# astooke/accel_rl

Measured on AMD Instinct MI355X. Metric: env-steps/sec (whole node), 256-env PPO Atari, higher is better.
Workload: dtype f32; 1 GPU; PPO breakout, 256 envs/GPU, horizon 5, spec-1 CNN (fp32), minibatch 512/GPU x 4 epochs, adam; synthetic fixed-frame emulator; hipGraph rollout; total_envs=256, global_minibatch=512, parallelism=single

## Files before the change

### accel_rl_amd/_lib.py

```python
import ctypes as C
import os

import torch

_PKG = os.path.dirname(os.path.abspath(__file__))
LIB_PATH = os.path.join(_PKG, "libaccel_rl_hip.so")

ARL_ABI_VERSION = 4
PROMO_NEP50, PROMO_LEGACY, PROMO_ASSOC = 0, 1, 2
PPO_TIE_THEANO, PPO_TIE_MATH, PPO_TIE_BOTH = 0, 1, 2
OPT_ADAM, OPT_RMSPROP = 0, 1
MAX_ACTIONS = 18
REPLAY_MAX_HORIZON = 16
RAW_H, RAW_W, OBS_H, OBS_W = 210, 160, 104, 80
OPT_PARTIALS = 1024

_vp, _i32, _i64, _f32, _f64 = C.c_void_p, C.c_int32, C.c_int64, C.c_float, C.c_double


class ArlGame(C.Structure):
    _fields_ = [("bank", _vp), ("n_frames", _i32), ("n_actions", _i32),
                ("action_set", _i32 * MAX_ACTIONS), ("start_lives", _i32),
                ("life_period", _i32), ("frame_skip", _i32), ("n_stack", _i32),
                ("clip_reward", _i32), ("episodic_lives", _i32), ("resample_mode", _i32)]
# ... 37 lines not shown
    _fields_ = [("part", _vp), ("out", _vp), ("total", _i64), ("splits", _i32), ("valid", _i32)]


FOLD_MAX_ITEMS = 24


class ArlLogitSrc(C.Structure):
    _fields_ = [("part", _vp), ("bias_or_null", _vp), ("split_stride", _i64), ("splits", _i32), ("reserved", _i32)]


class ArlDgradWt(C.Structure):
    _fields_ = [("w", _vp), ("wt", _vp), ("geom", C.POINTER(ArlConvGeom))]


DGRAD_WT_MAX = 4


class ArlServeHead(C.Structure):
    _fields_ = [("hidden", ArlFoldItem), ("hidden_bias", _vp), ("hidden_relu", _i32), ("hid", _i32),
                ("w_head", _vp), ("b_head", _vp)]


class ArlServeConv1(C.Structure):
    _fields_ = [("geom", C.POINTER(ArlConvGeom)), ("w", _vp), ("bias", _vp), ("y", _vp), ("scale", _f32),
                ("relu", _i32)]


class ArlNoisyLayer(C.Structure):
    _fields_ = [("fein", _vp), ("feout", _vp), ("x", _vp), ("xs", _vp), ("fan_in", _i32), ("units", _i32),
                ("out_stride", _i32), ("layer", _i32)]
# ... 38 lines not shown
    "arl_sample_categorical": (_i32, [_vp, _vp, _i64, _i32, _vp, _vp]),
    "arl_env_act_step": (_i32, [C.POINTER(ArlGame), C.POINTER(ArlEnvState), C.POINTER(ArlRollout),
                                _vp, _vp, _vp, _vp, _i32, _i32, _f64, _f64, _vp]),
    "arl_env_frame_step": (_i32, [C.POINTER(ArlGame), C.POINTER(ArlEnvState), C.POINTER(ArlRollout),
                                  _i32, _i32, _vp]),
    "arl_env_step": (_i32, [C.POINTER(ArlGame), C.POINTER(ArlEnvState), C.POINTER(ArlRollout),
                            _vp, _vp, _vp, _vp, _i32, _i32, _f64, _f64, _i32, _i32, _vp]),
    "arl_rollout_begin": (_i32, [C.POINTER(ArlGame), C.POINTER(ArlEnvState), C.POINTER(ArlRollout), _vp]),
    "arl_env_reset": (_i32, [C.POINTER(ArlGame), C.POINTER(ArlEnvState), C.POINTER(ArlRollout),
                             _vp, _i32, _vp]),
    "arl_preprocess_frames": (_i32, [_vp, _vp, _i64, _i32, _vp, _vp]),
    "arl_copy_bytes": (_i32, [_vp, _vp, _i64, _vp]),
    "arl_ring_append": (_i32, [_vp, _i32, _vp, _i32, _vp, _vp]),
    "arl_gather_scale_obs": (_i32, [_vp, _vp, _i64, _i64, _f32, _vp, _vp]),
    "arl_gather_scale_obs_nhwc": (_i32, [_vp, _vp, _i64, _i32, _i32, _f32, _vp, _vp]),
    "arl_traj_minibatch": (_i32, [_vp, _i32, _i32, _i64, C.POINTER(_vp), _i32, _i32, _vp, _vp, C.POINTER(_vp), _vp, _vp]),
    "arl_bias_relu": (_i32, [_vp, _vp, _i64, _i32, _vp]),
    "arl_relu_bwd_workspace_bytes": (_i64, []),
    "arl_relu_bwd_bias_grad": (_i32, [_vp, _vp, _i64, _i32, _vp, _vp, _vp]),
    "arl_pg_head_workspace_bytes": (_i64, []),
    "arl_pg_head_infer": (_i32, [_vp, _vp, _vp, _i64, _i32, _i32, _vp, _vp, _vp]),
    "arl_pg_head_loss": (_i32, [_vp] * 11 + [_i64, _i32, _i32, _i32, _i32, _f32, _f32, _f32, _i32] + [_vp] * 7),
    "arl_pg_head_loss_parts": (_i32, [_vp] * 11 + [_i64, _i32, _i32, _i32, _i32, _f32, _f32, _f32, _i32] + [_vp] * 7 +
                               [_vp, _i32, _vp]),
    "arl_conv_workspace_bytes": (_i64, []),
    "arl_conv2d_fwd": (_i32, [_vp, _vp, _vp, _vp, C.POINTER(ArlConvGeom), _i32, _vp, _vp]),
    "arl_conv2d_bwd_data": (_i32, [_vp, _vp, _vp, _vp, _vp, C.POINTER(ArlConvGeom), C.POINTER(ArlCorunJob), C.POINTER(_i32), _vp]),
    "arl_conv2d_dgrad_weights": (_i32, [C.POINTER(ArlDgradWt), _i32, _vp]),
    "arl_conv2d_bwd_weight": (_i32, [_vp, _vp, _vp, C.POINTER(ArlConvGeom), _vp, _vp]),
    "arl_conv2d_bwd_weight_parts": (_i32, [_vp, _vp, _vp, C.POINTER(ArlConvGeom), _vp, _i64, C.POINTER(ArlFoldItem),
# ... 349 lines not shown


def gather_scale_obs_nhwc(obs, idx, out, scale, stream=None):
    _want(obs, torch.uint8, "obs")
    _want(out, torch.float32, "out")
    if idx is not None:
        _want(idx, torch.int32, "idx")
    batch = out.shape[0]
    channels, plane = obs.shape[1], obs.shape[2] * obs.shape[3]
    assert out.numel() == batch * channels * plane
    _check(load().arl_gather_scale_obs_nhwc(ptr(obs), ptr(idx), batch, channels, plane, float(scale),
                                            out.data_ptr(), stream_ptr(stream)),
           "arl_gather_scale_obs_nhwc")


def traj_minibatch(seg, horizon, state_in, valids, idx, state_out, inv_count=None, stream=None):
    _want(seg, torch.int32, "seg")
    _want(idx, torch.int32, "idx")
    n_seg, n_state = seg.numel(), len(state_in)
    if len(state_out) != n_state:
        raise ValueError("traj_minibatch: %d states in, %d out" % (n_state, len(state_out)))
    if idx.numel() != n_seg * horizon:
        raise ValueError("traj_minibatch: idx holds %d rows, not %d segments x %d" % (idx.numel(), n_seg, horizon))
    hidden, total = 0, None
    for a, b in zip(state_in, state_out):
        _want(a, torch.float32, "state_in")
        _want(b, torch.float32, "state_out")
        hidden = a.shape[-1]
        if b.numel() != n_seg * hidden or a.numel() % (hidden * horizon) or total not in (None, a.numel() // hidden):
            raise ValueError("traj_minibatch: state shapes %s -> %s" % (tuple(a.shape), tuple(b.shape)))
# ... 649 lines not shown
```

### accel_rl_amd/algos/pg/aac_base.py

```python
import torch

from accel_rl_amd import _lib
from accel_rl_amd.algos.base import RLAlgorithm
from accel_rl_amd.buffers import buffer_with_segs_view
from accel_rl_amd.util import logger
from accel_rl_amd.util.misc import graph_capture_mode
from accel_rl_amd.util.quick_args import save_args
import numpy as np

LR_SCHEDULES = ["linear"]


def valids_mean(expression, valids=None):
    if valids is None:
        return expression.mean()
    v = valids.to(expression.dtype)
    return torch.sum(v * expression) * (1. / torch.sum(v))


class AdvActorCriticBase(RLAlgorithm):

    def __init__(self, discount, gae_lambda, v_loss_coeff=1, ent_loss_coeff=0.01,
                 standardize_adv=False, lr_schedule=None, promo="nep50", use_graph=True, bptt_resets=False):
        if lr_schedule is not None and lr_schedule not in LR_SCHEDULES:
# ... 41 lines not shown
            raise TypeError("the policy must provide loss_and_grads (HIP forward / backward into its flat "
                            "gradient bucket); got {}".format(type(policy).__name__))
        extra = dict(horizon=horizon, data_length=sample_size) if traj_opt else dict()
        self.optimizer.initialize(inputs=input_names, losses=self._losses, constraints=None, target=policy,
                                  lr_mult=self._lr_mult, **extra)
        self._opt_buf = buffer_with_segs_view(opt_examples, sample_size, horizon, dev)
        self._batch_size = sample_size
        self._mid_batch_reset = mid_batch_reset
        self._horizon = horizon
        self._n_env = sample_size // horizon
        self._std_ws = _lib.standardize_workspace(dev)
        self._lr_mult_host = torch.ones(1, dtype=torch.float32).pin_memory()
        self._graph = None
        self._graph_out = None
        self._graph_samples = None
        self._warm_calls = 0
        self._done_event = None
        self._info_ring = None
        self._info_replays = 0

    def set_n_itr(self, n_itr):
        self.n_itr = n_itr

    def optimize_policy(self, itr, samples_data):
        if self._done_event is not None:
            self._done_event.synchronize()
        if self.lr_schedule == "linear":
            self._lr_mult_host.fill_(max((self.n_itr - itr) / self.n_itr, 0.))
        if hasattr(self.optimizer, "prepare_host"):
            self.optimizer.prepare_host(self._batch_size)
# ... 5 lines not shown

    def _enqueue_optimize(self, itr, samples_data):
        tag = self.optimizer.parallelism_tag
        sync = tag == "synchronous" and getattr(self.optimizer, "graph_ready", lambda: False)()
        graphable = self.use_graph and hasattr(self.optimizer, "device_updates") and (tag == "single" or sync)
        if not graphable:
            return self._device_optimize(itr, samples_data)
        if self._graph is None:
            self._warm_calls += 1
            if self._warm_calls <= 2:
                out = self._device_optimize(itr, samples_data)
                self._ensure_info_ring(out[1])
                return out
            torch.cuda.synchronize(self.policy.device)
            graph, failure = torch.cuda.CUDAGraph(), None
            opt_host = {k: getattr(self.optimizer, k) for k in
                        ("_n_updates", "_hole", "_call_hole", "_hole_count", "_pending_avg") if hasattr(self.optimizer, k)}
            try:
                with torch.cuda.graph(graph, capture_error_mode=graph_capture_mode()):
                    self._graph_out = self._device_optimize(itr, samples_data)
                    self._append_infos(self._graph_out[1])
            except Exception as e:
                if not sync:
                    raise
                failure = e
            if sync and not self.optimizer.ranks_agree(failure is None):
                logger.log("WARNING: hipGraph capture of the synchronous learner failed on a rank (%r): eager "
                           "minibatches from here on" % (failure,))
                self.optimizer.graph_collectives = False
                for k, v in opt_host.items():
                    setattr(self.optimizer, k, v)
                torch.cuda.synchronize(self.policy.device)
                return self._device_optimize(itr, samples_data)
            self._graph, self._graph_samples = graph, samples_data
        assert samples_data is self._graph_samples, "the sampler must hand over the same buffer"
        self._graph.replay()
        opt_data, infos = self._graph_out
        slot = self._info_replays % next(iter(self._info_ring.values())).shape[0]
        self._info_replays += 1
        return opt_data, {k: self._info_ring[k][slot] for k in infos}

    INFO_RING = 4096
    _log_interval_itrs = 0

    def set_log_interval_itrs(self, n):
        self._log_interval_itrs = int(n)
        ring = getattr(self, "_info_ring", None)
        if ring is not None and self._ring_slots() > next(iter(ring.values())).shape[0]:
            raise RuntimeError("set_log_interval_itrs(%d) after the diagnostics ring was sized" % n)

    def _ring_slots(self):
        return max(self.INFO_RING, self._log_interval_itrs + 2)

    def _ensure_info_ring(self, infos):
        if self._info_ring is None:
# ... 77 lines not shown
```

### accel_rl_amd/csrc/batch_ops.hip

```cpp

#include <stdarg.h>
#include <string.h>

#include "arl_common.h"

namespace arl {
static thread_local char g_err[512] = "";
void set_error(const char* fmt, ...) {
    va_list ap;
    va_start(ap, fmt);
    vsnprintf(g_err, sizeof(g_err), fmt, ap);
    va_end(ap);
}
}

extern "C" int arl_abi_version(void) { return ARL_ABI_VERSION; }
extern "C" const char* arl_last_error(void) { return arl::g_err; }

namespace {

constexpr int STD_BLOCKS = 512;

__device__ __forceinline__ double wave_sum(double x) {
#pragma unroll
// ... 76 lines not shown
    const int64_t stride = (int64_t)gridDim.x * blockDim.x;
    for (int64_t i = (int64_t)blockIdx.x * blockDim.x + threadIdx.x; i < total; i += stride) {
        const int64_t b = i / row_vec, q = i - b * row_vec;
        const int64_t src_row = idx ? (int64_t)idx[b] : b;
        const uint4 w = reinterpret_cast<const uint4*>(obs)[src_row * row_vec + q];
        const uint32_t ws[4] = {w.x, w.y, w.z, w.w};
        float4* o = reinterpret_cast<float4*>(out) + i * 4;
#pragma unroll
        for (int k = 0; k < 4; ++k) {
            o[k] = make_float4((float)(ws[k] & 255u) * scale, (float)((ws[k] >> 8) & 255u) * scale,
                               (float)((ws[k] >> 16) & 255u) * scale, (float)(ws[k] >> 24) * scale);
        }
    }
}

}

extern "C" int64_t arl_standardize_workspace_bytes(void) { return (int64_t)STD_BLOCKS * 3 * sizeof(double); }

extern "C" int arl_standardize(float* advantages, const int8_t* valids_or_null, int64_t n,
                               double eps, void* workspace, void* stream) {
    ARL_REQUIRE(advantages && workspace, ARL_E_ARG, "null pointer");
    ARL_REQUIRE(n >= 0, ARL_E_ARG, "negative n");
    if (n == 0) return 0;
    hipStream_t s = (hipStream_t)stream;
    int64_t nb = (n + 255) / 256;
    if (nb > STD_BLOCKS) nb = STD_BLOCKS;
    hipLaunchKernelGGL(moments_kernel, dim3((unsigned)nb), dim3(256), 0, s, advantages,
                       valids_or_null, n, (double*)workspace);
    int rc = arl::check_launch("moments_kernel");
// ... 64 lines not shown
    return arl::check_launch("copy_kernel");
}

extern "C" int arl_gather_scale_obs(const uint8_t* obs, const int32_t* idx_or_null, int64_t batch,
                                    int64_t row_bytes, float scale, float* out, void* stream) {
    ARL_REQUIRE(obs && out, ARL_E_ARG, "null pointer");
    ARL_REQUIRE(batch >= 0 && row_bytes > 0, ARL_E_ARG, "bad batch/row_bytes");
    ARL_REQUIRE((row_bytes & 15) == 0, ARL_E_RANGE, "row_bytes must be a multiple of 16");
    ARL_REQUIRE(arl::aligned16(obs) && arl::aligned16(out), ARL_E_ALIGN, "obs/out must be 16-byte aligned");
    if (batch == 0) return 0;
    const int64_t row_vec = row_bytes >> 4;
    hipLaunchKernelGGL(gather_scale_kernel, dim3(arl::stream_grid(batch * row_vec, 256)), dim3(256),
                       0, (hipStream_t)stream, obs, idx_or_null, batch, row_vec, scale, out);
    return arl::check_launch("gather_scale_kernel");
}
```

### accel_rl_amd/optimizers/base.py

```python
import numpy as np
import torch

from accel_rl_amd import _lib

NORM_LOG_LEN = 64


def iterate_mb_idxs(batch_size, data_length, shuffle=False):
    if shuffle:
        order = np.arange(data_length)
        np.random.shuffle(order)
    for lo in range(0, data_length - batch_size + 1, batch_size):
        yield order[lo:lo + batch_size] if shuffle else np.arange(lo, lo + batch_size)


def iterate_traj_idxs(batch_size, data_length, horizon=1, shuffle=False):
    if data_length % horizon or batch_size % horizon or data_length % batch_size:
        raise AssertionError("batch_size and data_length must be multiples of horizon, data_length of batch_size")
    rows = np.arange(data_length).reshape(-1, horizon)
    order = np.arange(data_length // horizon)
    per = batch_size // horizon
    if shuffle:
        np.random.shuffle(order)
    for lo in range(0, len(order), per):
# ... 34 lines not shown
        st = _lib.ArlOptState()
        st.n_params = n
        st.params, st.grads = target.flat_params.data_ptr(), target.flat_grads.data_ptr()
        st.slot0 = self._slot0.data_ptr()
        st.slot1 = self._slot1.data_ptr() if self._slot1 is not None else None
        st.step_count, st.lr_mult = self._step_count.data_ptr(), self._lr_mult.data_ptr()
        st.partials, st.grad_norm_log = self._partials.data_ptr(), self._norm_log.data_ptr()
        st.norm_log_len = NORM_LOG_LEN
        self._opt_state = st
        a = self._update_args
        if self._update_method.name == "adam":
            self._kernel_args = (a["beta1"], a["beta2"], a["epsilon"])
        else:
            self._kernel_args = (a["rho"], 0.0, a["epsilon"])

    def _backward(self, losses, minibatch):
        return losses(minibatch)[3]

    def _apply_update(self, avg_factor=1.0):
        b1, b2, eps = self._kernel_args
        if self._grad_norm_clip is None:
            self._noclip_state()
            k = self._n_updates % self._opt_state.norm_log_len
            hole, self._hole = self._hole, None
            if k == 0:
                self._call_hole = hole
                self._hole_count = hole[1] if hole else 0
            elif self._hole_count and hole is None:
                hole = self._call_hole
                _lib.corun_job_run(_lib.corun_job(self._opt_state, self._update_method.kernel_id, self._learning_rate,
                                                  avg_factor, b1, b2, eps, k, self._step_pp, self._norm_parts,
                                                  hole[0], hole[1]))
            if self._hole_count:
                hole = self._call_hole
                _lib.opt_step_noclip_split(self._opt_state, self._update_method.kernel_id, self._learning_rate,
                                           avg_factor, b1, b2, eps, k, self._step_pp, self._norm_parts, hole[0],
                                           hole[1], 0)
            else:
                _lib.opt_step_noclip(self._opt_state, self._update_method.kernel_id, self._learning_rate, avg_factor,
                                     b1, b2, eps, k, self._step_pp, self._norm_parts)
            self._pending_avg = avg_factor
        else:
            _lib.opt_step(self._opt_state, self._update_method.kernel_id, self._learning_rate,
                          avg_factor, self._grad_norm_clip, b1, b2, eps)
        self._n_updates += 1

    corun_update = True

    def _noclip_state(self):
        if self._step_pp is None:
            dev = self._target.device
            self._step_pp = self._step_count.repeat(2).contiguous()
            self._norm_parts = torch.zeros(_lib.OPT_NORM_SLOTS * _lib.OPT_NORM_BLOCKS, dtype=torch.float64, device=dev)
        elif self._n_updates % self._opt_state.norm_log_len == 0 and not self._hole:
            self._step_pp.copy_(self._step_count.expand(2))

    def _corun_hook(self, avg_factor=1.0):
        if self._grad_norm_clip is not None or not self.corun_update:
            return None
        b1, b2, eps = self._kernel_args
# ... 28 lines not shown
```

### accel_rl_amd/optimizers/single.py

```python
import numpy as np
import torch

from accel_rl_amd import _lib

from accel_rl_amd.optimizers.base import BaseOptimizer, iterate_mb_idxs, iterate_traj_idxs


class A2cOptimizer(BaseOptimizer):

    def __init__(self, learning_rate, update_method, update_method_args=None, grad_norm_clip=None):
        self._learning_rate = learning_rate
        self._update_method = update_method
        self._update_args = update_method.resolve(**(update_method_args or dict()))
        self._grad_norm_clip = grad_norm_clip

    def initialize(self, inputs, losses, constraints, target, givens=None, lr_mult=1):
        self._input_names = list(inputs)
        self._losses = losses
        self._setup_bucket(target, lr_mult, givens)

    def optimize(self, inputs):
        self.prepare_host(len(inputs[0]))
        return self.device_updates(inputs)

    def prepare_host(self, data_length):
        self._set_updates_per_call(1)

    def device_updates(self, inputs):
        minibatch = dict(zip(self._input_names, inputs))
        minibatch["idx"] = None
        loss = self._backward(self._losses, minibatch)
        self._share_grad()
        self._apply_update(self._avg_factor())
        return loss, self._recent_grad_norms(1)

    def _share_grad(self):
        pass

    def _avg_factor(self):
        return 1.0

    @property
    def parallelism_tag(self):
        return "single"

# ... 33 lines not shown
        if flat:
            self._idx_host.copy_(torch.from_numpy(np.stack(flat).astype(np.int32)))

    def device_updates(self, inputs):
        data = dict(zip(self._input_names, inputs))
        if not self._n_minibatches:
            return [], []
        _lib.copy_bytes(self._idx_dev, self._idx_host)
        if self._overlap_allreduce:
            return self._overlapped_minibatches(data)
        losses = []
        corun = self._corun_hook() if self.parallelism_tag == "single" else None
        try:
            for k in range(self._n_minibatches):
                mb = self._minibatch(data, self._idx_dev[k])
                if corun is not None:
                    mb["dense_w_hook"] = corun
                losses.append(self._backward(self._losses, mb))
                self._share_grad()
                self._apply_update(self._avg_factor())
        finally:
            self._hole = None
        return losses, self._recent_grad_norms(self._n_minibatches)

    def _minibatch(self, data, idx):
        return dict(data, idx=idx)

    _overlap_allreduce = False

    def _overlapped_minibatches(self, data):
# ... 80 lines not shown
```

### accel_rl_amd/policies/atari_cnn_policy.py

```python
import ctypes as C
import os

import numpy as np
import torch

from accel_rl_amd import _lib
from accel_rl_amd.distributions import Categorical
from accel_rl_amd.spaces import Discrete
from accel_rl_amd.util.seed import layer_rng

KIND_A2C, KIND_PPO = 0, 1


def _glorot_uniform(shape):
    receptive = int(np.prod(shape[2:]))
    fan_in, fan_out = shape[1] * receptive, shape[0] * receptive
    a = np.sqrt(6. / (fan_in + fan_out))
    return layer_rng().uniform(low=-a, high=a, size=shape).astype(np.float32)


def _norm_c(shape, std):
    out = np.random.randn(*shape).astype(np.float32)
    out *= std / np.sqrt(np.square(out).sum(axis=0, keepdims=True))
    return out


class ObsRows(object):
    __slots__ = ("obs", "idx", "shape")

    def __init__(self, obs, idx):
        self.obs, self.idx = obs.contiguous(), idx
        self.shape = (obs.shape[0] if idx is None else idx.shape[0],) + tuple(obs.shape[1:])


class AtariCnnPolicy(object):

    _u8_conv1 = True
    serves_rows = True

    def __init__(self, conv_filters, conv_filter_sizes, conv_strides, conv_pads,
                 hidden_sizes=(), pixel_scale=255., initial_param_values=None):
        self.conv_filters, self.conv_filter_sizes = list(conv_filters), list(conv_filter_sizes)
        self.conv_strides, self.conv_pads = list(conv_strides), list(conv_pads)
        self.hidden_sizes = list(hidden_sizes)
        if not self.hidden_sizes:
            raise NotImplementedError("at least one hidden dense layer is required")
        self.pixel_scale = pixel_scale
# ... 61 lines not shown
        def views(flat):
            out = []
            for k, (o, n, s) in enumerate(zip(self._offsets, sizes, shapes)):
                v = flat[o:o + n].view(s)
                out.append(v.permute(0, 3, 1, 2) if (len(s) == 4 and not (k == 0 and self._u8)) else v)
            return out
        self.params = [torch.nn.Parameter(v) for v in views(self.flat_params)]
        self.grads = views(self.flat_grads)
        self._w = [self.flat_params[o:o + n] for o, n in zip(self._offsets, sizes)]
        self._g = [self.flat_grads[o:o + n] for o, n in zip(self._offsets, sizes)]
        self._conv_ws = _lib.conv_workspace(self.device)
        self._wt = {i: torch.empty_like(self._w[2 * i]) for i, (nf, ci, sz, st, pad, ho, wo) in enumerate(self._conv_geom)
                    if i > 0 and 16 < ci <= 64 and st <= 2 and sz % st == 0 and
                    os.environ.get("ARL_DGRAD_WT", "1") != "0"}
        self._geoms = dict()
        for p, g in zip(self.params, self.grads):
            p.grad = g
        self._n_conv, self._n_hid = len(self._conv_geom), len(self._hid_geom)
        self._dist = Categorical(n_act)
        self._scale = float(np.float32(1. / self.pixel_scale))
        self._relu_ws = _lib.relu_bwd_workspace(self.device)
        self._folds, self._fold_workspaces = _lib.FoldList(), {}
        self._loss_ws = _lib.pg_head_workspace(self.device)
        self._set_from_reference_arrays(ref)
        if self.initial_param_values is not None:
            self.set_param_values(self.initial_param_values)

    def _hidden_reference_init(self, fan):
        ref, names, self._hid_geom = [], [], []
        for i, hs in enumerate(self.hidden_sizes):
# ... 127 lines not shown

    def prob_value(self, observations, rows=None):
        with torch.no_grad():
            x = self._scaled(observations, rows)
            b = x.shape[0]
            _, hids = self._trunk(x)
            prob = torch.empty((b, self.n_act), dtype=torch.float32, device=self.device)
            value = torch.empty(b, dtype=torch.float32, device=self.device)
            _lib.pg_head_infer(hids[-1], self.params[-2], self.params[-1], prob, value)
            return prob, value

    def serve_supported(self):
        return (type(self).prob_value is AtariCnnPolicy.prob_value and self._n_hid >= 1 and
                self._hid_geom[-1][0] <= 1024 and self.n_act <= _lib.MAX_ACTIONS)

    def serve_conv1(self, game, b):
        conv_g, _ = self._layer_geoms(b)
        if not (self._u8 and _lib.serve_conv1_supported(game, conv_g[0])):
            return None, None
        nf, ci, sz, st, pad, ho, wo = self._conv_geom[0]
        y1 = self._buffer(("act", 0, b), (b, ho, wo, nf))
        conv1 = _lib.ArlServeConv1()
        conv1.geom = C.pointer(conv_g[0])
        conv1.w, conv1.bias, conv1.y = self._w[0].data_ptr(), self._w[1].data_ptr(), y1.data_ptr()
        conv1.scale, conv1.relu = self._scale, 1
        return conv1, y1

    def serve_forward(self, game, observations, rows, y1=None, want_next=True):
        with torch.no_grad():
            b = rows.shape[0]
            conv_g, dense_g = self._layer_geoms(b)
            w = self._w
            nf, ci, sz, st, pad, ho, wo = self._conv_geom[0]
            if y1 is None:
                x = self._scaled(observations, rows)
                y1 = self._buffer(("act", 0, b), (b, ho, wo, nf))
                if isinstance(x, ObsRows):
                    _lib.conv2d_u8_fwd(x.obs, x.idx, self._scale, w[0], w[1], y1, conv_g[0], True)
                else:
                    _lib.conv2d_fwd(x, w[0], w[1], y1, conv_g[0], True, self._conv_ws)
            a = y1
            for i in range(1, self._n_conv):
                nf_i, _, _, _, _, ho_i, wo_i = self._conv_geom[i]
                z = self._buffer(("act", i, b), (b, ho_i, wo_i, nf_i))
                _lib.conv2d_fwd(a, w[2 * i], w[2 * i + 1], z, conv_g[i], True, self._conv_ws)
                a = z
            k = 2 * self._n_conv
            for j, (hs, fan_in) in enumerate(self._hid_geom):
                hcur = self._buffer(("hid", j, b), (b, hs))
                if j + 1 < self._n_hid:
                    _lib.conv2d_fwd(a, w[k], w[k + 1], hcur, dense_g[j], True, self._conv_ws)
                else:
                    item = _lib.conv2d_fwd_parts(a, w[k], w[k + 1], hcur, dense_g[j], True, self._conv_ws)
                a = hcur
                k += 2
            head = _lib.ArlServeHead()
            head.hidden = item
            head.hidden_bias, head.hidden_relu, head.hid = w[k - 1].data_ptr(), 1, self._hid_geom[-1][0]
            head.w_head, head.b_head = w[self._k_head].data_ptr(), w[self._k_head + 1].data_ptr()
            conv1 = None
            if want_next and self._u8 and _lib.serve_conv1_supported(game, conv_g[0]):
                conv1 = _lib.ArlServeConv1()
                conv1.geom = C.pointer(conv_g[0])
                conv1.w, conv1.bias, conv1.y = w[0].data_ptr(), w[1].data_ptr(), y1.data_ptr()
                conv1.scale, conv1.relu = self._scale, 1
            return head, conv1, (y1 if conv1 is not None else None)

    def loss_and_grads(self, mb, kind, clip_param, v_loss_coeff, ent_loss_coeff, lr_mult,
                       inv_count=None, tie_rule=_lib.PPO_TIE_THEANO):
        with torch.no_grad():
            idx = mb.get("idx")
            rows = mb["observations"].shape[0] if idx is None else idx.shape[0]
            limit = self.rows_per_pass()
            if limit and rows >= 3 * limit:
                return self._loss_and_grads_in_passes(mb, rows, limit, kind, clip_param, v_loss_coeff, ent_loss_coeff,
                                                      lr_mult, inv_count, tie_rule)
            x = self._scaled(mb["observations"], idx)
            b = x.shape[0]
            acts, hids = self._trunk(x)
            g, k_head = self.grads, self._k_head
            hid = self._hid_geom[-1][0]
            dout = self._buffer(("dout", b), (b, self.n_act + 1))
            dh = self._buffer(("dh", b), (b, hid))
            loss4 = self._buffer(("loss", b), (4,))
            wts = self._dgrad_weight_items(b) if os.environ.get("ARL_WT_IN_HEAD", "1") != "0" else []
            self._folds.pg_head_loss(hids[-1], self.params[k_head], self.params[k_head + 1], mb["actions"],
                              mb["advantages"], mb["returns"], mb.get("old_prob"), mb.get("valids"),
                              idx, lr_mult, inv_count, self.n_act, kind, clip_param, v_loss_coeff,
                              ent_loss_coeff, dout, dh, g[k_head], g[k_head + 1], loss4, self._loss_ws,
                              relu_mask_dh=True, tie_rule=tie_rule, dgrad_weights=wts)
            self._wt_fresh = bool(wts)
            try:
                self._backward_trunk(x, acts, hids, dh, masked=True, split_hook=mb.get("split_hook"),
                                     dense_w_hook=mb.get("dense_w_hook"))
# ... 178 lines not shown
        for i in range(self._n_conv):
            w = ref[k][:, :, ::-1, ::-1]
            if not (i == 0 and self._u8):
                w = w.transpose(0, 2, 3, 1)
            if i == 0 and not self._u8 and self._c_pad != self._c_in:
                w = np.concatenate([w, np.zeros(w.shape[:3] + (self._c_pad - self._c_in,), np.float32)], axis=3)
            internal += [w, ref[k + 1]]
            k += 2
        tail = self._tail_from_flat(list(ref[k:]))
        internal += self._hidden_to_internal(tail[:self._n_hidden_tensors])
        internal += self._head_to_internal(tail[self._n_hidden_tensors:])
        for o, s, a in zip(self._offsets, self._shapes, internal):
            assert tuple(a.shape) == tuple(s), (a.shape, s)
            host[o:o + a.size] = np.ascontiguousarray(a).reshape(-1)
        self.flat_params.copy_(torch.from_numpy(host))

    def set_param_values(self, flat, trainable=True):
        flat = np.asarray(flat, np.float32)
        assert flat.size == self.n_params
        ref, pos = [], 0
        for s in self._ref_shapes:
            n = int(np.prod(s))
            ref.append(flat[pos:pos + n].reshape(s))
            pos += n
        self._set_from_reference_arrays(ref)
```

### accel_rl_amd/runners/sync.py

```python
import os
import time

import torch
import torch.distributed as dist

from accel_rl_amd.runners.accel_rl import AccelRL
from accel_rl_amd.util import logger


class AccelRLSync(AccelRL):

    def __init__(self, affinities=None, seed=None, backend=None, **kwargs):
        self._backend = backend
        self._worker_affinities = None
        self._worker_procs = []
        as_list = list(affinities) if isinstance(affinities, (list, tuple)) else None
        if "WORLD_SIZE" in os.environ:
            self.rank = int(os.environ.get("RANK", 0))
            self.n_runners = int(os.environ["WORLD_SIZE"])
            if as_list is not None:
                if len(as_list) != self.n_runners:
                    raise ValueError("AccelRLSync got %d affinities but WORLD_SIZE=%d: one entry per launched rank "
                                     "(multigpu_rl_base.py:21)" % (len(as_list), self.n_runners))
                affinities = as_list[self.rank]
# ... 134 lines not shown
        n_itr = super().startup(master=True)
        self.init_comm()
        self._start_time = self._last_time = time.time()
        return n_itr

    def init_comm(self):
        if self.n_runners > 1:
            n = torch.tensor([self.policy.flat_params.numel()], dtype=torch.int64, device=self.policy.flat_params.device)
            lo, hi = n.clone(), n.clone()
            dist.all_reduce(lo, op=dist.ReduceOp.MIN)
            dist.all_reduce(hi, op=dist.ReduceOp.MAX)
            if int(lo) != int(hi):
                raise ValueError("AccelRLSync: the runners' policies differ in size (%d ... %d parameters, %d here): a "
                                 "synchronous clique all-reduces ONE flat bucket" % (int(lo), int(hi), int(n)))
            dist.broadcast(self.policy.flat_params, src=0)
            self._initial_param_vector = self.policy.flat_params.clone()
        self.algo.optimizer.init_comm(None, self.rank, self.n_runners)
        if self.n_runners > 1:
            dist.barrier()

    def get_n_itr(self, sample_size):
        n_itr = super().get_n_itr(sample_size * self.n_runners)
        return n_itr

    def store_diagnostics(self, itr, samples_data, opt_data, traj_infos, opt_infos):
        if self.n_runners > 1 and (itr + 1) % self._log_interval_itrs == 0:
            pending = getattr(self, "_pending_traj", []) + list(traj_infos)
            gathered = [None] * self.n_runners
            dist.all_gather_object(gathered, [dict(t) for t in pending])
            self._pending_traj = []
# ... 16 lines not shown
```

### accel_rl_amd/sampler/gpu_sampler.py

```python
import ctypes
import os

import numpy as np
import torch

from accel_rl_amd import _lib
from accel_rl_amd.buffers import (buffer_with_segs_view, batch_buffer, combine_distinct_buffers,
                                  buffer_length, count_buffer_size)
from accel_rl_amd.envs import synthetic_atari as synth
from accel_rl_amd.sampler.base import BaseMbSampler
from accel_rl_amd.sampler.util import TrajInfo
from accel_rl_amd.util import logger
from accel_rl_amd.util.misc import graph_capture_mode, nbytes_unit, struct

NOOP_RING = 4096


def _packed_block(spec, device, pinned=False):
    offsets, total = [], 0
    for _, shape, dtype in spec:
        total = (total + 127) // 128 * 128
        offsets.append(total)
        total += int(np.prod(shape)) * torch.empty((), dtype=dtype).element_size()
    block = torch.zeros(total, dtype=torch.uint8, device=device)
# ... 41 lines not shown
    def __eq__(self, other):
        self.resolve()
        return super().__eq__(other)

    def __repr__(self):
        self.resolve()
        return super().__repr__()


class GpuVecSampler(BaseMbSampler):

    _alias_extra_obs = True
    _serve_in_step = os.environ.get("ARL_SERVE_IN_STEP", "1") != "0"
    _serve_in_step_max_envs = (512, 1024)
    _two_host_sets = os.environ.get("ARL_TWO_HOST_SETS", "1") != "0"

    def __init__(self, n_parallel=1, envs_per=1, device=None, use_graph=True, **kwargs):
        super().__init__(n_parallel=n_parallel, envs_per=envs_per, **kwargs)
        self._total_n_envs = 2 * n_parallel * envs_per
        self.device = device
        self.use_graph = use_graph
        self._sets, self._batch_no = [], 0

    @property
    def _graph(self):
        return self._sets[0].graph if self._sets else None

    @_graph.setter
    def _graph(self, value):
        for h in self._sets:
# ... 133 lines not shown
                agent_infos[key] = np.zeros(state.shape[1], np.float32)
            self._prev_frozen = torch.zeros(n, dtype=torch.uint8, device=dev)
        examples = dict(actions=np.zeros((), self.env_spec.action_space.dtype), agent_infos=agent_infos)
        policy_buf = buffer_with_segs_view(examples, n * t, t, dev)
        self.samples_buf = combine_distinct_buffers(self.envs_buf, policy_buf)
        assert buffer_length(self.samples_buf) == self.sample_size
        policy.reset(n_batch=n if self._recurrent else self.n_parallel * self.envs_per)
        self._rollout = self._make_rollout(self.samples_buf)
        self._single_write = bool(self.mid_batch_reset and not self._recurrent and
                                  getattr(policy, "serves_rows", False) and self._kernel_max_path_length() >= 1)
        self._serve_fused = bool(self._single_write and type(self)._serve_in_step and self._game.n_stack <= 4 and
                                 hasattr(policy, "serve_forward") and policy.serve_supported())
        if self._serve_fused:
            with_conv1 = policy.serve_conv1(self._game, n)[0] is not None
            self._serve_fused = n <= type(self)._serve_in_step_max_envs[int(with_conv1)]
        self._extra_is_step_obs = bool(self.need_extra_obs and self.mid_batch_reset and type(self)._alias_extra_obs)
        if self._extra_is_step_obs:
            self.samples_buf.extra_observations = self.envs_buf.extra_observations = self.step_obs
        self._step_rows = (torch.arange(n, dtype=torch.int32, device=dev)[None, :] * t +
                           torch.arange(t, dtype=torch.int32, device=dev)[:, None]).contiguous()
        self._uniforms = torch.empty((t, n), dtype=torch.float64, device=dev)
        self._sets, self._batch_no, self._last_pending = [], 0, None
        overlap = (self.use_graph and type(self)._two_host_sets and not hasattr(policy, "host_draws") and not self._recurrent)
        for _ in range(2 if overlap else 1):
            block, views = _packed_block(self._results_spec, "cpu", pinned=True)
            self._sets.append(struct(uniforms_host=torch.empty(t * n, dtype=torch.float64).pin_memory(), host_block=block,
                                     host=struct(**views), event=torch.cuda.Event(), pending=None, graph=None))
        logger.log("GpuVecSampler -- total_n_envs: {}".format(self.total_n_envs))
        logger.log("GpuVecSampler -- batch buffer size: {:,.1f} {}".format(
            *nbytes_unit(count_buffer_size(self.samples_buf))))
# ... 2 lines not shown
        n, t = self._total_n_envs, self.horizon
        cur = self._sets[self._batch_no % len(self._sets)]
        self._batch_no += 1
        if cur.pending is not None:
            cur.pending.resolve()
        draws = self.policy.host_draws(t, n) if hasattr(self.policy, "host_draws") else np.random.rand(t * n)
        cur.uniforms_host.copy_(torch.from_numpy(draws))
        with torch.cuda.device(self.device):
            if self.use_graph:
                if cur.graph is None:
                    self._capture(cur)
                cur.graph.replay()
            else:
                self._enqueue_batch(cur)
            cur.event.record()
        older = self._last_pending if (self._last_pending is not None and self._last_pending._sampler is not None) else None
        cur.pending = self._last_pending = _LazyTrajInfos(self, cur, older)
        return self.samples_buf, cur.pending

    def shutdown(self):
        for h in self._sets:
            h.graph = None

    @property
    def alternating(self):
        return False

    def _make_rollout(self, buf):
        ro = _lib.ArlRollout()
        ro.horizon = self.horizon
        ro.step_obs = self.step_obs.data_ptr()
        if buf is not None:
            ro.observations = buf.observations.data_ptr()
            ro.rewards, ro.dones = buf.rewards.data_ptr(), buf.dones.data_ptr()
            ro.raw_reward = buf.env_infos["raw_reward"].data_ptr() if "raw_reward" in buf.env_infos else None
            ro.need_reset = buf.env_infos["need_reset"].data_ptr() if "need_reset" in buf.env_infos else None
            ro.actions = buf.actions.data_ptr()
            ro.prob, ro.value = buf.agent_infos["prob"].data_ptr(), buf.agent_infos["value"].data_ptr()
        return ro

    def _enqueue_batch(self, cur):
        n, t = self._total_n_envs, self.horizon
        buf, ro, env = self.samples_buf, self._rollout, self.env
        _lib.copy_bytes(self._uniforms, cur.uniforms_host)
        conv1, y1 = self.policy.serve_conv1(self._game, n) if self._serve_fused else (None, None)
        if conv1 is not None:
            _lib.rollout_begin_conv1(self._game, self._state, ro, conv1)
        else:
            _lib.rollout_begin(self._game, self._state, ro)
        for s in range(t):
            if hasattr(self.policy, "set_step"):
                self.policy.set_step(s)
            if self._serve_fused:
                head, conv1, y1 = self.policy.serve_forward(self._game, buf.observations, self._step_rows[s], y1,
                                                            want_next=s + 1 < t)
                _lib.env_step_served(self._game, self._state, ro, head, conv1, self._uniforms[s], s,
                                     self._kernel_max_path_length(), self.discount, env.max_start_noops)
                continue
            if self._recurrent:
                prob, value, *prev = self.policy.act_step(self.step_obs)
                for key, state in zip(self.policy.state_info_keys, prev):
                    buf.agent_infos[key].view(n, t, -1)[:, s].copy_(state)
                if not self.mid_batch_reset:
                    self._prev_frozen.copy_(self._st.frozen)
            elif self._single_write:
                prob, value = self.policy.prob_value(buf.observations, self._step_rows[s])
            else:
                prob, value = self.policy.prob_value(self.step_obs)
            self._env_step(self._state, ro, prob, value, self._uniforms[s], s, self.mid_batch_reset,
                           single_write=self._single_write)
# ... 116 lines not shown
```

### include/accel_rl_hip.h

```cpp
#ifndef ACCEL_RL_HIP_H
#define ACCEL_RL_HIP_H

#include <stdint.h>

#ifdef __cplusplus
extern "C" {
#endif

#define ARL_ABI_VERSION 4

#define ARL_E_ARG      (-1)
#define ARL_E_RANGE    (-2)
#define ARL_E_ALIGN    (-3)

#define ARL_PROMO_NEP50   0
#define ARL_PROMO_LEGACY  1
#define ARL_PROMO_ASSOC   2

int         arl_abi_version(void);
const char* arl_last_error(void);


int arl_gae_scan(const float* rewards, const float* values, const uint8_t* dones,
                 const float* last_values, double discount, double gae_lambda,
// ... 110 lines not shown

int arl_preprocess_frames(const uint8_t* raw_a_or_null, const uint8_t* raw_b,
                          int64_t n, int32_t resample_mode, uint8_t* out, void* stream);


int arl_copy_bytes(void* dst, const void* src, int64_t nbytes, void* stream);
int arl_ring_append(const float* src, int32_t n, float* ring, int32_t n_slots, int32_t* counter, void* stream);

int arl_gather_scale_obs(const uint8_t* obs, const int32_t* idx_or_null, int64_t batch,
                         int64_t row_bytes, float scale, float* out, void* stream);

int arl_gather_scale_obs_nhwc(const uint8_t* obs, const int32_t* idx_or_null, int64_t batch,
                              int32_t channels, int32_t plane_bytes, float scale, float* out,
                              void* stream);

int arl_traj_minibatch(const int32_t* seg, int32_t n_seg, int32_t horizon, int64_t n_traj_total,
                       const float* const* state_in, int32_t n_state, int32_t hidden,
                       const int8_t* valids_or_null, int32_t* idx, float* const* state_out,
                       float* inv_count_or_null, void* stream);

int arl_bias_relu(float* x, const float* bias, int64_t rows, int32_t channels, void* stream);

int64_t arl_relu_bwd_workspace_bytes(void);
int arl_relu_bwd_bias_grad(float* dy, const float* y, int64_t rows, int32_t channels,
                           float* dbias, void* workspace, void* stream);
typedef struct arl_fold_item {
    const float* part;
    float*       out;
    int64_t      total;
    int32_t      splits;
// ... 391 lines not shown
```

Before: 363,700 env-steps/s.

## Reuse rollout conv activations for the first PPO minibatch forward pass

```diff
diff --git a/accel_rl_amd/_lib.py b/accel_rl_amd/_lib.py
--- a/accel_rl_amd/_lib.py
+++ b/accel_rl_amd/_lib.py
@@ -75,6 +75,13 @@
 
 
 DGRAD_WT_MAX = 4
+
+
+class ArlGatherItem(C.Structure):
+    _fields_ = [("src", _vp), ("dst", _vp), ("floats_per_row", _i64)]
+
+
+GATHER_MAX_ITEMS = 8
 
 
 class ArlServeHead(C.Structure):
@@ -143,6 +150,7 @@
     "arl_ring_append": (_i32, [_vp, _i32, _vp, _i32, _vp, _vp]),
     "arl_gather_scale_obs": (_i32, [_vp, _vp, _i64, _i64, _f32, _vp, _vp]),
     "arl_gather_scale_obs_nhwc": (_i32, [_vp, _vp, _i64, _i32, _i32, _f32, _vp, _vp]),
+    "arl_gather_act_rows": (_i32, [_vp, _i64, _i64, _i32, _vp, _i32, _vp]),
     "arl_traj_minibatch": (_i32, [_vp, _i32, _i32, _i64, C.POINTER(_vp), _i32, _i32, _vp, _vp, C.POINTER(_vp), _vp, _vp]),
     "arl_bias_relu": (_i32, [_vp, _vp, _i64, _i32, _vp]),
     "arl_relu_bwd_workspace_bytes": (_i64, []),
@@ -522,6 +530,29 @@
            "arl_gather_scale_obs_nhwc")
 
 
+def gather_act_rows(idx, n_env, horizon, items, stream=None):
+    if not 0 < len(items) <= GATHER_MAX_ITEMS:
+        raise ValueError("gather_act_rows: 1 .. %d items" % GATHER_MAX_ITEMS)
+    rows = items[0][1].shape[0]
+    if idx is not None:
+        _want(idx, torch.int32, "idx")
+        if idx.numel() != rows:
+            raise ValueError("gather_act_rows: %d indices for %d rows" % (idx.numel(), rows))
+    arr = (ArlGatherItem * len(items))()
+    for k, (src, dst) in enumerate(items):
+        _want(src, torch.float32, "src")
+        _want(dst, torch.float32, "dst")
+        per = dst[0].numel() if rows else 0
+        if dst.shape[0] != rows or src.dim() < 2 or src.shape[1] != n_env or src.shape[0] < horizon or \
+                src[0, 0].numel() != per:
+            raise ValueError("gather_act_rows: store %s does not hold [%d+][%d] rows of the %s destination" %
+                             (tuple(src.shape), horizon, n_env, tuple(dst.shape)))
+        arr[k].src, arr[k].dst, arr[k].floats_per_row = ptr(src), ptr(dst), per
+    if rows:
+        _check(load().arl_gather_act_rows(ptr(idx), rows, n_env, horizon, arr, len(items), stream_ptr(stream)),
+               "arl_gather_act_rows")
+
+
 def traj_minibatch(seg, horizon, state_in, valids, idx, state_out, inv_count=None, stream=None):
     _want(seg, torch.int32, "seg")
     _want(idx, torch.int32, "idx")
diff --git a/accel_rl_amd/algos/pg/aac_base.py b/accel_rl_amd/algos/pg/aac_base.py
--- a/accel_rl_amd/algos/pg/aac_base.py
+++ b/accel_rl_amd/algos/pg/aac_base.py
@@ -79,6 +79,8 @@
         self._graph = None
         self._graph_out = None
         self._graph_samples = None
+        self._graph_reuses = False
+        self._graph_plain = None
         self._warm_calls = 0
         self._done_event = None
         self._info_ring = None
@@ -114,6 +116,7 @@
                 return out
             torch.cuda.synchronize(self.policy.device)
             graph, failure = torch.cuda.CUDAGraph(), None
+            uses = self._stored_acts_uses()
             opt_host = {k: getattr(self.optimizer, k) for k in
                         ("_n_updates", "_hole", "_call_hole", "_hole_count", "_pending_avg") if hasattr(self.optimizer, k)}
             try:
@@ -133,12 +136,36 @@
                 torch.cuda.synchronize(self.policy.device)
                 return self._device_optimize(itr, samples_data)
             self._graph, self._graph_samples = graph, samples_data
+            self._graph_reuses = self._stored_acts_uses() > uses
+            if self._graph_reuses:
+                plain = torch.cuda.CUDAGraph()
+                self.optimizer.offer_stored_acts = False
+                try:
+                    with torch.cuda.graph(plain, capture_error_mode=graph_capture_mode()):
+                        out = self._device_optimize(itr, samples_data)
+                        self._append_infos(out[1])
+                finally:
+                    self.optimizer.offer_stored_acts = True
+                self._graph_plain = (plain, out)
         assert samples_data is self._graph_samples, "the sampler must hand over the same buffer"
-        self._graph.replay()
-        opt_data, infos = self._graph_out
+        graph, self._graph_out_used = self._graph, self._graph_out
+        if self._graph_reuses and self.policy.stored_acts(samples_data["observations"]) is None:
+            graph, self._graph_out_used = self._graph_plain
+        graph.replay()
+        self._params_replayed()
+        opt_data, infos = self._graph_out_used
         slot = self._info_replays % next(iter(self._info_ring.values())).shape[0]
         self._info_replays += 1
         return opt_data, {k: self._info_ring[k][slot] for k in infos}
+
+    def _stored_acts_uses(self):
+        count = getattr(self.policy, "stored_acts_uses", None)
+        return count() if count is not None else 0
+
+    def _params_replayed(self):
+        changed = getattr(self.policy, "params_changed", None)
+        if changed is not None:
+            changed()
 
     INFO_RING = 4096
     _log_interval_itrs = 0
diff --git a/accel_rl_amd/csrc/batch_ops.hip b/accel_rl_amd/csrc/batch_ops.hip
--- a/accel_rl_amd/csrc/batch_ops.hip
+++ b/accel_rl_amd/csrc/batch_ops.hip
@@ -114,6 +114,41 @@
     }
 }
 
+constexpr int GA_CHUNK = 1024;
+struct GatherActArgs {
+    arl_gather_item items[ARL_GATHER_MAX_ITEMS];
+    int64_t task_start[ARL_GATHER_MAX_ITEMS + 1];
+    int chunks[ARL_GATHER_MAX_ITEMS];
+    int n;
+};
+
+__global__ __launch_bounds__(256) void gather_act_rows_kernel(const GatherActArgs a, const int32_t* __restrict__ idx,
+                                                              int64_t rows, int64_t n_env, int horizon) {
+    const int64_t n_tasks = a.task_start[a.n];
+    for (int64_t task = blockIdx.x; task < n_tasks; task += gridDim.x) {
+        int it = 0;
+        while (it + 1 < a.n && task >= a.task_start[it + 1]) ++it;
+        const int64_t local = task - a.task_start[it];
+        const int chunks = a.chunks[it];
+        const int64_t b = local / chunks;
+        const int c = (int)(local - b * chunks);
+        const int64_t r = idx ? (int64_t)idx[b] : b;
+        if (b >= rows || r < 0 || r >= n_env * horizon) continue;
+        const int64_t e = r / horizon, t = r - e * horizon;
+        const int64_t vec = a.items[it].floats_per_row >> 2;
+        const uint4* __restrict__ src = reinterpret_cast<const uint4*>(a.items[it].src) + (t * n_env + e) * vec;
+        uint4* __restrict__ dst = reinterpret_cast<uint4*>(a.items[it].dst) + b * vec;
+        const int64_t q0 = (int64_t)c * GA_CHUNK + threadIdx.x;
+        uint4 v[4];
+#pragma unroll
+        for (int k = 0; k < 4; ++k)
+            if (q0 + 256 * k < vec) v[k] = src[q0 + 256 * k];
+#pragma unroll
+        for (int k = 0; k < 4; ++k)
+            if (q0 + 256 * k < vec) dst[q0 + 256 * k] = v[k];
+    }
+}
+
 }
 
 extern "C" int64_t arl_standardize_workspace_bytes(void) { return (int64_t)STD_BLOCKS * 3 * sizeof(double); }
@@ -208,3 +243,28 @@
                        0, (hipStream_t)stream, obs, idx_or_null, batch, row_vec, scale, out);
     return arl::check_launch("gather_scale_kernel");
 }
+
+extern "C" int arl_gather_act_rows(const int32_t* idx_or_null, int64_t rows, int64_t n_env, int32_t horizon,
+                                   const arl_gather_item* items, int32_t n_items, void* stream) {
+    ARL_REQUIRE(items, ARL_E_ARG, "null pointer");
+    ARL_REQUIRE(rows >= 0 && n_env > 0 && horizon > 0, ARL_E_ARG, "bad rows / n_env / horizon");
+    ARL_REQUIRE(n_items > 0 && n_items <= ARL_GATHER_MAX_ITEMS, ARL_E_RANGE, "1 .. ARL_GATHER_MAX_ITEMS items");
+    ARL_REQUIRE(idx_or_null || rows <= n_env * horizon, ARL_E_RANGE, "without idx: at most n_env * horizon rows");
+    if (rows == 0) return 0;
+    GatherActArgs a = {};
+    a.n = n_items;
+    for (int i = 0; i < n_items; ++i) {
+        ARL_REQUIRE(items[i].src && items[i].dst, ARL_E_ARG, "null item pointer");
+        ARL_REQUIRE(items[i].floats_per_row > 0 && (items[i].floats_per_row & 3) == 0, ARL_E_RANGE,
+                    "floats_per_row must be a positive multiple of 4");
+        ARL_REQUIRE(arl::aligned16(items[i].src) && arl::aligned16(items[i].dst), ARL_E_ALIGN, "src/dst must be 16-byte aligned");
+        a.items[i] = items[i];
+        a.chunks[i] = (int)(((items[i].floats_per_row >> 2) + GA_CHUNK - 1) / GA_CHUNK);
+        a.task_start[i + 1] = a.task_start[i] + rows * a.chunks[i];
+    }
+    const int64_t n_tasks = a.task_start[n_items];
+    const unsigned grid = (unsigned)(n_tasks < 8192 ? n_tasks : 8192);
+    hipLaunchKernelGGL(gather_act_rows_kernel, dim3(grid), dim3(256), 0, (hipStream_t)stream, a, idx_or_null, rows, n_env,
+                       (int)horizon);
+    return arl::check_launch("gather_act_rows_kernel");
+}
diff --git a/accel_rl_amd/optimizers/base.py b/accel_rl_amd/optimizers/base.py
--- a/accel_rl_amd/optimizers/base.py
+++ b/accel_rl_amd/optimizers/base.py
@@ -72,6 +72,22 @@
         else:
             self._kernel_args = (a["rho"], 0.0, a["epsilon"])
 
+    def _offer_stored_acts(self, minibatch):
+        lookup = getattr(self._target, "stored_acts", None)
+        if lookup is None or not self.offer_stored_acts or self.parallelism_tag != "single" or \
+                "observations" not in minibatch:
+            return
+        handle = lookup(minibatch["observations"])
+        if handle is not None:
+            minibatch["stored_acts"] = handle
+
+    offer_stored_acts = True
+
+    def _params_written(self):
+        changed = getattr(self._target, "params_changed", None)
+        if changed is not None:
+            changed()
+
     def _backward(self, losses, minibatch):
         return losses(minibatch)[3]
 
@@ -102,6 +118,7 @@
             _lib.opt_step(self._opt_state, self._update_method.kernel_id, self._learning_rate,
                           avg_factor, self._grad_norm_clip, b1, b2, eps)
         self._n_updates += 1
+        self._params_written()
 
     corun_update = True
 
diff --git a/accel_rl_amd/optimizers/single.py b/accel_rl_amd/optimizers/single.py
--- a/accel_rl_amd/optimizers/single.py
+++ b/accel_rl_amd/optimizers/single.py
@@ -29,6 +29,7 @@
     def device_updates(self, inputs):
         minibatch = dict(zip(self._input_names, inputs))
         minibatch["idx"] = None
+        self._offer_stored_acts(minibatch)
         loss = self._backward(self._losses, minibatch)
         self._share_grad()
         self._apply_update(self._avg_factor())
@@ -92,6 +93,8 @@
         try:
             for k in range(self._n_minibatches):
                 mb = self._minibatch(data, self._idx_dev[k])
+                if k == 0:
+                    self._offer_stored_acts(mb)
                 if corun is not None:
                     mb["dense_w_hook"] = corun
                 losses.append(self._backward(self._losses, mb))
diff --git a/accel_rl_amd/policies/atari_cnn_policy.py b/accel_rl_amd/policies/atari_cnn_policy.py
--- a/accel_rl_amd/policies/atari_cnn_policy.py
+++ b/accel_rl_amd/policies/atari_cnn_policy.py
@@ -31,6 +31,13 @@
     def __init__(self, obs, idx):
         self.obs, self.idx = obs.contiguous(), idx
         self.shape = (obs.shape[0] if idx is None else idx.shape[0],) + tuple(obs.shape[1:])
+
+
+class ActStore(object):
+    __slots__ = ("convs", "n_env", "horizon", "stamp", "reused")
+
+    def __init__(self, convs, n_env, horizon):
+        self.convs, self.n_env, self.horizon, self.stamp, self.reused = convs, n_env, horizon, None, 0
 
 
 class AtariCnnPolicy(object):
@@ -122,6 +129,7 @@
                     if i > 0 and 16 < ci <= 64 and st <= 2 and sz % st == 0 and
                     os.environ.get("ARL_DGRAD_WT", "1") != "0"}
         self._geoms = dict()
+        self._act_stores, self._param_version = dict(), 0
         for p, g in zip(self.params, self.grads):
             p.grad = g
         self._n_conv, self._n_hid = len(self._conv_geom), len(self._hid_geom)
@@ -279,27 +287,29 @@
         return (type(self).prob_value is AtariCnnPolicy.prob_value and self._n_hid >= 1 and
                 self._hid_geom[-1][0] <= 1024 and self.n_act <= _lib.MAX_ACTIONS)
 
-    def serve_conv1(self, game, b):
+    def serve_conv1(self, game, b, store=None):
         conv_g, _ = self._layer_geoms(b)
         if not (self._u8 and _lib.serve_conv1_supported(game, conv_g[0])):
             return None, None
         nf, ci, sz, st, pad, ho, wo = self._conv_geom[0]
-        y1 = self._buffer(("act", 0, b), (b, ho, wo, nf))
+        assert store is None or store.n_env == b
+        y1 = store.convs[0][0] if store is not None else self._buffer(("act", 0, b), (b, ho, wo, nf))
         conv1 = _lib.ArlServeConv1()
         conv1.geom = C.pointer(conv_g[0])
         conv1.w, conv1.bias, conv1.y = self._w[0].data_ptr(), self._w[1].data_ptr(), y1.data_ptr()
         conv1.scale, conv1.relu = self._scale, 1
         return conv1, y1
 
-    def serve_forward(self, game, observations, rows, y1=None, want_next=True):
+    def serve_forward(self, game, observations, rows, y1=None, want_next=True, step=None, store=None):
         with torch.no_grad():
             b = rows.shape[0]
             conv_g, dense_g = self._layer_geoms(b)
             w = self._w
             nf, ci, sz, st, pad, ho, wo = self._conv_geom[0]
+            assert store is None or (store.n_env == b and 0 <= step < store.horizon - (1 if want_next else 0))
             if y1 is None:
                 x = self._scaled(observations, rows)
-                y1 = self._buffer(("act", 0, b), (b, ho, wo, nf))
+                y1 = store.convs[0][step] if store is not None else self._buffer(("act", 0, b), (b, ho, wo, nf))
                 if isinstance(x, ObsRows):
                     _lib.conv2d_u8_fwd(x.obs, x.idx, self._scale, w[0], w[1], y1, conv_g[0], True)
                 else:
@@ -307,7 +317,7 @@
             a = y1
             for i in range(1, self._n_conv):
                 nf_i, _, _, _, _, ho_i, wo_i = self._conv_geom[i]
-                z = self._buffer(("act", i, b), (b, ho_i, wo_i, nf_i))
+                z = store.convs[i][step] if store is not None else self._buffer(("act", i, b), (b, ho_i, wo_i, nf_i))
                 _lib.conv2d_fwd(a, w[2 * i], w[2 * i + 1], z, conv_g[i], True, self._conv_ws)
                 a = z
             k = 2 * self._n_conv
@@ -325,11 +335,66 @@
             head.w_head, head.b_head = w[self._k_head].data_ptr(), w[self._k_head + 1].data_ptr()
             conv1 = None
             if want_next and self._u8 and _lib.serve_conv1_supported(game, conv_g[0]):
+                y1 = store.convs[0][step + 1] if store is not None else y1
                 conv1 = _lib.ArlServeConv1()
                 conv1.geom = C.pointer(conv_g[0])
                 conv1.w, conv1.bias, conv1.y = w[0].data_ptr(), w[1].data_ptr(), y1.data_ptr()
                 conv1.scale, conv1.relu = self._scale, 1
             return head, conv1, (y1 if conv1 is not None else None)
+
+    def act_store_alloc(self, n_env, horizon):
+        key = (int(n_env), int(horizon))
+        if key in self._act_stores:
+            return self._act_stores[key]
+        ok = (os.environ.get("ARL_REUSE_ROLLOUT_ACTS", "1") != "0" and self.serve_supported() and self._u8 and
+              type(self)._trunk is AtariCnnPolicy._trunk and type(self).loss_and_grads is AtariCnnPolicy.loss_and_grads and
+              _lib.default_route in (_lib.ROUTE_SPLIT9, _lib.ROUTE_SPLIT6) and
+              all(nf <= 64 for nf, ci, sz, st, pad, ho, wo in self._conv_geom))
+        store = None
+        if ok:
+            store = ActStore([torch.zeros((horizon, n_env, ho, wo, nf), dtype=torch.float32, device=self.device)
+                              for nf, ci, sz, st, pad, ho, wo in self._conv_geom], key[0], key[1])
+        self._act_stores[key] = store
+        return store
+
+    def params_changed(self):
+        self._param_version += 1
+
+    def _params_stamp(self):
+        return (self._param_version, self.flat_params._version)
+
+    def act_store_stamp(self, store, observations):
+        store.stamp = (self._params_stamp(), observations.data_ptr(), observations._version)
+
+    def stored_acts(self, observations):
+        for store in self._act_stores.values():
+            if store is not None and self._store_valid(store, observations):
+                return store
+        return None
+
+    def stored_acts_uses(self):
+        return sum(store.reused for store in self._act_stores.values() if store is not None)
+
+    def _store_valid(self, store, observations):
+        return (isinstance(store, ActStore) and self._act_stores.get((store.n_env, store.horizon)) is store and
+                store.stamp == (self._params_stamp(), observations.data_ptr(), observations._version) and
+                observations.shape[0] == store.n_env * store.horizon and not self.rows_per_pass() and
+                _lib.default_route in (_lib.ROUTE_SPLIT9, _lib.ROUTE_SPLIT6))
+
+    def _trunk_from_store(self, store, idx, b):
+        conv_g, dense_g = self._layer_geoms(b)
+        acts = [self._buffer(("act", i, b), (b, ho, wo, nf))
+                for i, (nf, ci, sz, st, pad, ho, wo) in enumerate(self._conv_geom)]
+        _lib.gather_act_rows(idx, store.n_env, store.horizon, list(zip(store.convs, acts)))
+        store.reused += 1
+        hids, k, a, w = [], 2 * self._n_conv, acts[-1], self._w
+        for j, (hs, fan_in) in enumerate(self._hid_geom):
+            hcur = self._buffer(("hid", j, b), (b, hs))
+            _lib.conv2d_fwd(a, w[k], w[k + 1], hcur, dense_g[j], True, self._conv_ws)
+            hids.append(hcur)
+            a = hcur
+            k += 2
+        return acts, hids
 
     def loss_and_grads(self, mb, kind, clip_param, v_loss_coeff, ent_loss_coeff, lr_mult,
                        inv_count=None, tie_rule=_lib.PPO_TIE_THEANO):
@@ -342,7 +407,11 @@
                                                       lr_mult, inv_count, tie_rule)
             x = self._scaled(mb["observations"], idx)
             b = x.shape[0]
-            acts, hids = self._trunk(x)
+            store = mb.get("stored_acts")
+            if store is not None and self._store_valid(store, mb["observations"]):
+                acts, hids = self._trunk_from_store(store, idx, b)
+            else:
+                acts, hids = self._trunk(x)
             g, k_head = self.grads, self._k_head
             hid = self._hid_geom[-1][0]
             dout = self._buffer(("dout", b), (b, self.n_act + 1))
@@ -551,6 +620,7 @@
             assert tuple(a.shape) == tuple(s), (a.shape, s)
             host[o:o + a.size] = np.ascontiguousarray(a).reshape(-1)
         self.flat_params.copy_(torch.from_numpy(host))
+        self.params_changed()
 
     def set_param_values(self, flat, trainable=True):
         flat = np.asarray(flat, np.float32)
diff --git a/accel_rl_amd/runners/sync.py b/accel_rl_amd/runners/sync.py
--- a/accel_rl_amd/runners/sync.py
+++ b/accel_rl_amd/runners/sync.py
@@ -172,6 +172,8 @@
                 raise ValueError("AccelRLSync: the runners' policies differ in size (%d ... %d parameters, %d here): a "
                                  "synchronous clique all-reduces ONE flat bucket" % (int(lo), int(hi), int(n)))
             dist.broadcast(self.policy.flat_params, src=0)
+            if hasattr(self.policy, "params_changed"):
+                self.policy.params_changed()
             self._initial_param_vector = self.policy.flat_params.clone()
         self.algo.optimizer.init_comm(None, self.rank, self.n_runners)
         if self.n_runners > 1:
diff --git a/accel_rl_amd/sampler/gpu_sampler.py b/accel_rl_amd/sampler/gpu_sampler.py
--- a/accel_rl_amd/sampler/gpu_sampler.py
+++ b/accel_rl_amd/sampler/gpu_sampler.py
@@ -79,6 +79,7 @@
     _serve_in_step = os.environ.get("ARL_SERVE_IN_STEP", "1") != "0"
     _serve_in_step_max_envs = (512, 1024)
     _two_host_sets = os.environ.get("ARL_TWO_HOST_SETS", "1") != "0"
+    _act_store = None
 
     def __init__(self, n_parallel=1, envs_per=1, device=None, use_graph=True, **kwargs):
         super().__init__(n_parallel=n_parallel, envs_per=envs_per, **kwargs)
@@ -242,6 +243,8 @@
         if self._serve_fused:
             with_conv1 = policy.serve_conv1(self._game, n)[0] is not None
             self._serve_fused = n <= type(self)._serve_in_step_max_envs[int(with_conv1)]
+        self._act_store = (policy.act_store_alloc(n, t) if self._serve_fused and hasattr(policy, "act_store_alloc")
+                           else None)
         self._extra_is_step_obs = bool(self.need_extra_obs and self.mid_batch_reset and type(self)._alias_extra_obs)
         if self._extra_is_step_obs:
             self.samples_buf.extra_observations = self.envs_buf.extra_observations = self.step_obs
@@ -274,6 +277,8 @@
             else:
                 self._enqueue_batch(cur)
             cur.event.record()
+        if self._act_store is not None:
+            self.policy.act_store_stamp(self._act_store, self.samples_buf.observations)
         older = self._last_pending if (self._last_pending is not None and self._last_pending._sampler is not None) else None
         cur.pending = self._last_pending = _LazyTrajInfos(self, cur, older)
         return self.samples_buf, cur.pending
@@ -303,7 +308,13 @@
         n, t = self._total_n_envs, self.horizon
         buf, ro, env = self.samples_buf, self._rollout, self.env
         _lib.copy_bytes(self._uniforms, cur.uniforms_host)
-        conv1, y1 = self.policy.serve_conv1(self._game, n) if self._serve_fused else (None, None)
+        store = self._act_store
+        if not self._serve_fused:
+            conv1, y1 = None, None
+        elif store is not None:
+            conv1, y1 = self.policy.serve_conv1(self._game, n, store=store)
+        else:
+            conv1, y1 = self.policy.serve_conv1(self._game, n)
         if conv1 is not None:
             _lib.rollout_begin_conv1(self._game, self._state, ro, conv1)
         else:
@@ -312,8 +323,9 @@
             if hasattr(self.policy, "set_step"):
                 self.policy.set_step(s)
             if self._serve_fused:
+                kw = dict(step=s, store=store) if store is not None else dict()
                 head, conv1, y1 = self.policy.serve_forward(self._game, buf.observations, self._step_rows[s], y1,
-                                                            want_next=s + 1 < t)
+                                                            want_next=s + 1 < t, **kw)
                 _lib.env_step_served(self._game, self._state, ro, head, conv1, self._uniforms[s], s,
                                      self._kernel_max_path_length(), self.discount, env.max_start_noops)
                 continue
diff --git a/include/accel_rl_hip.h b/include/accel_rl_hip.h
--- a/include/accel_rl_hip.h
+++ b/include/accel_rl_hip.h
@@ -148,6 +148,15 @@
                               int32_t channels, int32_t plane_bytes, float scale, float* out,
                               void* stream);
 
+#define ARL_GATHER_MAX_ITEMS 8
+typedef struct {
+    const float* src;
+    float* dst;
+    int64_t floats_per_row;
+} arl_gather_item;
+int arl_gather_act_rows(const int32_t* idx_or_null, int64_t rows, int64_t n_env, int32_t horizon,
+                        const arl_gather_item* items, int32_t n_items, void* stream);
+
 int arl_traj_minibatch(const int32_t* seg, int32_t n_seg, int32_t horizon, int64_t n_traj_total,
                        const float* const* state_in, int32_t n_state, int32_t hidden,
                        const int8_t* valids_or_null, int32_t* idx, float* const* state_out,
```

Result: no change. 362,600 env-steps/s (-0.3%).
